# bobu36000/gym-chess

Measured on AMD Instinct MI355X. Metric: env steps/sec at 65 536 boards per GPU (random-policy self-play to terminal, auto-reset), higher is better.
Workload: dtype u64

## Files before the change

### __graft_entry__.py

```python
import os
import subprocess
import sys

ROOT = os.path.dirname(os.path.abspath(__file__))
PKG_DIR = os.path.join(ROOT, "gym-chess_amd")
LIB = os.path.join(PKG_DIR, "gym_chess_amd", "libgymchess.so")
CORE_HOST = os.path.join(ROOT, "tests", "core_host")


def _run(cmd):
    print("+", " ".join(cmd), flush=True)
    subprocess.run(cmd, check=True)


def _lib_module():
    sys.path.insert(0, PKG_DIR)
    from gym_chess_amd import _lib

    return _lib


def build_hip(force=False):
    L = _lib_module()
    want = L.source_hash()
    if not force and os.path.exists(LIB) and L.built_hash(LIB) == want:
        return
    tmp = LIB + ".tmp"
    _run(["hipcc"] + L.BUILD_FLAGS + [f'-DGC_SRC_HASH="{want}"', "-o", tmp,
                                      os.path.join(PKG_DIR, "csrc", "gymchess.hip")])
    os.replace(tmp, LIB)


def build_oracle():
    _run(["make", "-s", "-C", os.path.join(ROOT, "oracle")])


def build_core_host():
    sys.path.insert(0, CORE_HOST)
    import clonehost
    import corehost
    import rankfillhost

    corehost.ensure_built()
    rankfillhost.ensure_built()
    clonehost.ensure_built()


def build():
    build_hip()
    build_oracle()
    build_core_host()
    sys.path.insert(0, PKG_DIR)
    import gym_chess_amd
    from gym_chess_amd import _lib

    _lib.load()


def smoke():
    sys.path.insert(0, PKG_DIR)
    sys.path.insert(0, os.path.join(ROOT, "oracle"))
    import numpy as np

    import oracle as O
    from gym_chess_amd.engine import Engine
    from gym_chess_amd.env import BatchedChessEnv

    eng = Engine(0)
    b = np.tile(O.DEFAULT_BOARD, (64, 1))
    m = np.tile(O.make_meta(), (64, 1))
    nodes = eng.perft(b, m, 3)
    assert (nodes == 8982).all(), nodes[:4]
    moves, cnt = eng.possible_moves(b[:1], m[:1], True)
    assert [int(x) for x in moves[0, : cnt[0]]] == O.get_possible_moves(O.DEFAULT_BOARD, O.make_meta(), True)
    env = BatchedChessEnv(32, device=0, seed=7)
    _, tr = env.rollout(60, trace=True)
    for i in range(32):
        ref = O.rollout_trace(7, i, 60)
        assert (tr["action"][:, i] == ref["action"]).all(), f"board {i} actions differ"
        assert (tr["reward"][:, i] == ref["reward"]).all(), f"board {i} rewards differ"
        assert (tr["done"][:, i] == ref["done"]).all(), f"board {i} done differs"
    print("smoke ok: perft(3)=8982 x64, startpos list, 32x60-ply rollout == oracle", flush=True)


if __name__ == "__main__":
    build()
    if len(sys.argv) > 1 and sys.argv[1] == "smoke":
        smoke()
```

### gym-chess_amd/csrc/gc_core.h

```cpp
#pragma once
#include <type_traits>
#include <stdint.h>

#if defined(__HIPCC__)
#include <hip/hip_runtime.h>
#define GC_HD __host__ __device__ __forceinline__
#define GC_HDM __host__ __device__ __forceinline__
#else
#define GC_HD static inline
#define GC_HDM inline
#endif

namespace gc {

typedef uint64_t u64;
typedef uint32_t u32;

enum { EMPTY = 0, KING = 1, QUEEN = 2, ROOK = 3, BISHOP = 4, KNIGHT = 5, PAWN = 6 };
enum { A_KSW = 4096, A_QSW = 4097, A_KSB = 4098, A_QSB = 4099, A_RESIGN = 4100, A_NONE = 0xFFFF };

enum : u32 {
    M_WHITE = 1u, M_WKC = 2u, M_WQC = 4u, M_BKC = 8u, M_BQC = 16u, M_RIGHTS = 30u,
    M_WCHK = 32u, M_BCHK = 64u, M_DONE = 128u,
    M_MC_SHIFT = 8, M_MC_MASK = 0xFFu << 8,
// ... 1231 lines not shown
            return sq * 64 + (g.white ? sq - 9 : sq + 7);
        }
        return sq * 64 + kth_target(rtg, sq, type_at(s, sq), g.white, k);
    }
    if (g.castles & 1) { if (k == 0) return g.white ? A_QSW : A_QSB; k--; }
    if (g.castles & 2) { if (k == 0) return g.white ? A_KSW : A_KSB; }
    return A_NONE;
}

GC_HD bool action_legal(const Pos& s, const Gen& g, int action) {
    if (action < 0 || action > A_RESIGN) return false;
    if (action >= 4096) {
        if (g.white) return (action == A_QSW && (g.castles & 1)) || (action == A_KSW && (g.castles & 2));
        return (action == A_QSB && (g.castles & 1)) || (action == A_KSB && (g.castles & 2));
    }
    int f = action >> 6, t = action & 63;
    if (!((g.own >> f) & 1)) return false;
    return (legal_targets(s, g, f, type_at(s, f)) >> t) & 1;
}

GC_HD bool quick_legal(const Pos& s, int action) {
    if (action < 0 || action > A_RESIGN) return false;
    Gen g;
    gen_base(s, g);
    if (action >= 4096) {
        gen_enemy(s, g);
        return action_legal(s, g, action);
    }
    const int f = action >> 6, t = action & 63;
    if (!((g.own >> f) & 1)) return false;
    const int ty = type_at(s, f);
    if (ty == KING) return ((king_set(bit(f)) & ~g.own) >> t & 1) && !sq_attacked(s, t, !g.white);
    gen_pins(s, g);
    return (legal_targets(s, g, f, ty) >> t) & 1;
}

GC_HD bool quick_pseudo(const Pos& s, int action) {
    if (action < 0 || action > A_RESIGN) return false;
    Gen g;
    gen_base(s, g);
    if (action >= 4096) {
        gen_enemy(s, g);
        return action_legal(s, g, action);
    }
    const int f = action >> 6, t = action & 63;
    const u64 fb = bit(f), tb = bit(t);
    const int ty = type_at(s, f);
    const int df = (t & 7) - (f & 7), dr = (t >> 3) - (f >> 3);
    const bool orth = (df == 0) != (dr == 0);
    const bool dia = df != 0 && (df == dr || df == -dr);
    const bool clear = (between(f, t) & g.occ) == 0;
    const u64 empty = ~g.occ;
    const u64 push = g.white ? (((fb >> 8) | ((fb & ROW6) >> 16)) & empty) : (((fb << 8) | ((fb & ROW1) << 16)) & empty);
    const u64 pawn = push | (pawn_att_set(fb, g.white) & g.opp);
    const u64 leap = (ty == KNIGHT ? knight_set(fb) : king_set(fb)) & ~g.own;
    const bool ok = ty == PAWN ? (pawn & tb) != 0
                  : (ty == KNIGHT || ty == KING) ? (leap & tb) != 0
                  : ty == QUEEN ? (orth || dia) && clear
                  : ty == ROOK ? orth && clear
                  : ty == BISHOP ? dia && clear : false;
    return ((g.own >> f) & 1) && ok && (ty == PAWN || !(g.own & tb));
}
GC_HD bool quick_safe(const Pos& s, int action) {
    if (action < 0 || action >= 4096) return true;
    const int f = action >> 6, t = action & 63;
    Gen g;
    gen_base(s, g);
    if (type_at(s, f) == KING) return !sq_attacked(s, t, !g.white);
    gen_pins(s, g);
    if (g.ks < 0) return true;
    u64 tg = g.checkmask;
    if (g.pinned & bit(f)) tg &= g.pinrays & line_through(g.ks, f) & king_side(g.ks, f);
    return (tg >> t) & 1;
}

GC_HD int apply_move(Pos& s, bool white_player, int action, int* reward, bool* irrev) {
    *reward = 0;
    *irrev = false;
    if (action < 4096) {
        int f = action >> 6, t = action & 63;
        int pid = id_at(s, f);
        if (pid == 0) return -1;
        int cid = id_at(s, t);
        int pt = pid < 0 ? -pid : pid, ct = cid < 0 ? -cid : cid;
        clear_sq(s, f);
        clear_sq(s, t);
        int nid = pid;
        *reward = (int)((0x1335A00u >> (4 * ct)) & 0xFu);
        if (pt == PAWN && ((white_player && (t >> 3) == 7) || (!white_player && (t >> 3) == 0))) {
            nid = white_player ? QUEEN : -QUEEN;
            *reward += 10;
        }
        put(s, t, nid);
        *irrev = (pt == PAWN) || (cid != 0);
        if (pid == KING) {
            s.meta &= white_player ? ~(u32)(M_WKC | M_WQC) : ~(u32)(M_BKC | M_BQC);
        } else if (pid == ROOK) {
            if ((f & 7) == 0) s.meta &= white_player ? ~(u32)M_WQC : ~(u32)M_BQC;
            else if ((f & 7) == 7) s.meta &= white_player ? ~(u32)M_WKC : ~(u32)M_BKC;
        }
    } else {
        switch (action) {
            case A_KSW:
                clear_sq(s, 60); clear_sq(s, 61); clear_sq(s, 62); clear_sq(s, 63);
                put(s, 61, ROOK); put(s, 62, KING);
                s.meta &= ~(u32)(M_WKC | M_WQC);
                break;
            case A_QSW:
                clear_sq(s, 56); clear_sq(s, 57); clear_sq(s, 58); clear_sq(s, 59); clear_sq(s, 60);
                put(s, 58, KING); put(s, 59, ROOK);
                s.meta &= ~(u32)(M_WKC | M_WQC);
                break;
            case A_KSB:
                clear_sq(s, 4); clear_sq(s, 5); clear_sq(s, 6); clear_sq(s, 7);
                put(s, 5, -ROOK); put(s, 6, -KING);
                s.meta &= ~(u32)(M_BKC | M_BQC);
                break;
            case A_QSB:
                clear_sq(s, 0); clear_sq(s, 1); clear_sq(s, 2); clear_sq(s, 3); clear_sq(s, 4);
                put(s, 2, -KING); put(s, 3, -ROOK);
                s.meta &= ~(u32)(M_BKC | M_BQC);
                break;
            default: return -2;
        }
    }
    s.meta = white_player ? (s.meta & ~(u32)M_WHITE) : (s.meta | M_WHITE);
    return 0;
}

GC_HD void apply_legal_with(Pos& s, bool white, int action, int* reward, bool* irrev, u64 occ0, u64 kw, u64 rw) {
    const bool cs = action >= 4096;
    const bool cw = action == A_KSW || action == A_QSW, cks = action == A_KSW || action == A_KSB;
    const int base = cw ? 56 : 0;
    const u64 cclr = cks ? (0xFull << (base + 4)) : (0x1Full << base);
    const u64 ck = cs ? bit(base + (cks ? 6 : 2)) : 0ull, cr = cs ? bit(base + (cks ? 5 : 3)) : 0ull;
    int f = (action >> 6) & 63, t = action & 63;
    u64 fm = cs ? 0ull : bit(f), tm = cs ? 0ull : bit(t), clr = cs ? ~cclr : ~(fm | tm);
    int v = 10 * (int)((s.q >> t) & 1) + 5 * (int)((s.r >> t) & 1) + 3 * (int)(((s.b | s.n) >> t) & 1) +
            (int)((s.p >> t) & 1);
    *reward = cs ? 0 : v;
    *irrev = !cs && (((s.p & fm) != 0) || ((occ0 & tm) != 0));
    bool wk = (kw & fm) != 0, wr = (rw & fm) != 0;
#define GC_MV(X) s.X = (s.X & clr) | ((s.X & fm) ? tm : 0ull)
    GC_MV(k); GC_MV(q); GC_MV(r); GC_MV(b); GC_MV(n); GC_MV(p); GC_MV(w);
#undef GC_MV
    s.k |= ck;
    s.r |= cr;
    s.w |= cw ? (ck | cr) : 0ull;
    u32 clear = (wk ? (u32)(M_WKC | M_WQC) : 0u) | ((wr && (f & 7) == 0) ? (u32)M_WQC : 0u) |
                ((wr && (f & 7) == 7) ? (u32)M_WKC : 0u);
    clear = cs ? (cw ? (u32)(M_WKC | M_WQC) : (u32)(M_BKC | M_BQC)) : clear;
    s.meta = (s.meta & ~clear) ^ M_WHITE;
}
GC_HD void apply_legal(Pos& s, bool white, int action, int* reward, bool* irrev) {
    apply_legal_with(s, white, action, reward, irrev, occ_of(s), s.k & s.w, s.r & s.w);
}

GC_HD u64 mix64(u64 x) {
    x ^= x >> 31; x *= 0x7FB5D329728EA185ull;
    x ^= x >> 27; x *= 0x81DADEF4BC2DD44Dull;
    x ^= x >> 33;
    return x;
}
GC_HD u64 rotl64(u64 x, int r) { return (x << r) | (x >> (64 - r)); }
GC_HD u32 rotl32(u32 x, int r) { return (x << r) | (x >> (32 - r)); }
GC_HD u32 board_key(const Pos& s) {
    const u64 x = s.k ^ rotl64(s.q, 11) ^ rotl64(s.r, 22) ^ rotl64(s.b, 37) ^ rotl64(s.n, 46) ^ rotl64(s.p, 55) ^
                  rotl64(s.w, 5);
    u32 y = ((u32)x * 0x9E3779B1u) ^ rotl32((u32)(x >> 32) * 0x85EBCA77u, 16);
    y ^= y >> 15;
    y *= 0x2C1B3C6Du;
    return y ^ (y >> 12);
}

GC_HD Pos from_mailbox(const int8_t* b, u32 meta) {
    Pos s = {0, 0, 0, 0, 0, 0, 0, meta};
    for (int i = 0; i < 64; i++) put(s, i, b[i]);
    return s;
}
GC_HD void to_mailbox(const Pos& s, int8_t* b) {
    for (int i = 0; i < 64; i++) b[i] = (int8_t)id_at(s, i);
}

GC_HD u32 philox_x0(u64 seed, u32 board, u32 draw) {
    u32 k0 = (u32)seed, k1 = (u32)(seed >> 32);
    u32 x0 = board, x1 = draw, x2 = 0x5EEDu, x3 = 0u;
#pragma unroll
    for (int i = 0; i < 10; i++) {
        u64 p0 = (u64)0xD2511F53u * x0;
        u64 p1 = (u64)0xCD9E8D57u * x2;
        u32 y0 = (u32)(p1 >> 32) ^ x1 ^ k0;
        u32 y1 = (u32)p1;
        u32 y2 = (u32)(p0 >> 32) ^ x3 ^ k1;
        u32 y3 = (u32)p0;
        x0 = y0; x1 = y1; x2 = y2; x3 = y3;
        k0 += 0x9E3779B9u;
        k1 += 0xBB67AE85u;
    }
    return x0;
}
GC_HD u32 scale_rank(u32 x0, u32 n) { return (u32)(((u64)x0 * n) >> 32); }
GC_HD u32 policy_index(u64 seed, u32 board, u32 draw, u32 n) { return scale_rank(philox_x0(seed, board, draw), n); }

}
```

### gym-chess_amd/csrc/gymchess.hip

```cpp
#include <hip/hip_runtime.h>
#include <hipcub/hipcub.hpp>

#include <cmath>
#include <cstdio>
#include <cstdlib>
#include <cstring>
#include <atomic>
#include <chrono>
#include <mutex>
#include <string>
#include <type_traits>
#include <vector>

#ifdef GC_STAMPS
__shared__ unsigned long long gc_stamp_lds[4][8];
__device__ __forceinline__ void gc_stamp(int k) {
    __builtin_amdgcn_sched_barrier(0);
    unsigned long long t;
#ifdef GC_STAMPS_REAL
    asm volatile("s_memrealtime %0\n\ts_waitcnt lgkmcnt(0)" : "=s"(t)::"memory");
    if (k == 0) {
        unsigned hw, xcc;
        asm volatile("s_getreg_b32 %0, hwreg(HW_REG_HW_ID)\n\ts_getreg_b32 %1, hwreg(HW_REG_XCC_ID)"
                     : "=s"(hw), "=s"(xcc));
// ... 1634 lines not shown
        } else {
            h.commit();
            io.store(i, s);
            h.flush(g0);
            io.nsteps[i] = nst;
            io.reward[i] = o.reward;
            io.done[i] = (uint8_t)o.done;
            io.reason[i] = (uint8_t)o.reason;
        }
    }
    GC_STAMP(7);
#ifdef GC_STAMPS
    if (g_stamp_out != nullptr && l == 0)
        for (int q = 0; q < 8; q++) g_stamp_out[((size_t)blk * 2 + role) * 8 + q] = gc_stamp_lds[threadIdx.x >> 6][q];
#endif
}


__device__ __forceinline__ u64 trace_word(int played, const StepOut& o) {
    return (u64)(uint16_t)(int16_t)played | ((u64)(uint16_t)(int16_t)o.reward << 16) | ((u64)(o.done & 0xFF) << 32) |
           ((u64)(o.reason & 0xFF) << 40);
}
#define ROLLOUT_MAX_PLIES 16383

#ifdef GC_PSTAMPS
__device__ __forceinline__ unsigned long long pst_entry_where() {
    const unsigned long long t = __builtin_amdgcn_s_memrealtime();
    unsigned hw, xcc;
    asm volatile("s_getreg_b32 %0, hwreg(HW_REG_HW_ID)\n\ts_getreg_b32 %1, hwreg(HW_REG_XCC_ID)" : "=s"(hw), "=s"(xcc));
    const unsigned long long where = ((hw >> 8) & 0xF) | (((hw >> 12) & 1) << 4) | (((hw >> 13) & 3) << 5) |
                                     (((hw >> 4) & 3) << 7) | ((unsigned long long)(xcc & 0xF) << 9);
    return (t & ((1ull << 44) - 1)) | (where << 44);
}
#endif

template <bool FIDE, int OPP = 0>
__global__ void __launch_bounds__(2 * PAIR_BOARDS * PAIRS_WG) PAIR_ATTR
    k_env_rollout2(uint8_t* __restrict__ slab, int nn, uint64_t seed, u64* __restrict__ htab,
                   const uint16_t* __restrict__ racts, const EnvDev::InitCache* __restrict__ icd, u32 rinfo,
                   uint64_t* __restrict__ stats, u64* __restrict__ trace) {
    constexpr bool API = false;
    constexpr int blk0 = 0;
    const int plies = (int)(rinfo >> 18);
    rinfo &= 0x1FFFFu;
#ifdef GC_PSTAMPS
    const unsigned long long g_pst_entry = pst_entry_where();
#endif
    PAIR_PROLOGUE
    uint64_t steps = 0, rsum = 0;
    u32 e_mate = 0, e_rep = 0, e_cap = 0, e_nomove = 0, e_err = 0;
    StepOut o = {0, 0, R_NONE, 0};
#ifdef GC_PSTAMPS
    unsigned long long rt0 = 0, rt1 = 0;
    if (l == 0) {
        for (int k = 0; k < 8; k++) gc_pst[threadIdx.x >> 6][k] = 0;
        gc_pst[threadIdx.x >> 6][8] = __builtin_amdgcn_s_memtime();
    }
    rt0 = __builtin_amdgcn_s_memrealtime();
#endif
    const int wg_half = ((nn + PAIR_BOARDS * PAIRS_WG - 1) / (PAIR_BOARDS * PAIRS_WG)) >> 1;
    auto plies_loop = [&](auto R, auto ST) {
        for (int p = 0; p < plies; p++) {
            int played = a;
            if (GC_PAIR_FAIR) {
                if ((((int)blockIdx.x >= wg_half) ? 1 : 0) ^ (p & 1)) __builtin_amdgcn_s_setprio(1);
                else __builtin_amdgcn_s_setprio(0);
            }
            o = pair_step<OPP, true, FIDE>(Ls, L, C, R, l, i, live, rp, s, a, d, h, nst);
#ifdef GC_PSTAMPS
            if (p == 0) rt1 = __builtin_amdgcn_s_memrealtime();
#endif
            if (R) {
                if (trace && live) trace[(size_t)p * nn + i] = trace_word(played == A_NONE ? -1 : played, o);
                if (!ST) {
                } else if (played == A_NONE) {
                    e_nomove++;
                } else {
                    steps++;
                    rsum += (uint64_t)(int64_t)o.reward;
                    if (o.done) {
                        e_mate += o.reason == R_MATE || o.reason == R_MATED;
                        e_rep += o.reason == R_REPETITION;
                        e_cap += o.reason == R_MOVE_CAP;
                        e_err += o.reason == R_BOTH_CHECKED || o.reason == R_WINDOW_FULL;
                        e_nomove += o.reason == R_OPP_NO_MOVE;
                    }
                }
                h.commit();
            }
        }
#ifdef GC_PSTAMPS
        if (g_pst_out != nullptr && l == 0) {
            const size_t w = (size_t)blockIdx.x * (blockDim.x >> 6) + (threadIdx.x >> 6);
            for (int k = 0; k < 8; k++) g_pst_out[w * 12 + k] = gc_pst[threadIdx.x >> 6][k];
            g_pst_out[w * 12 + 8] = g_pst_entry;
            g_pst_out[w * 12 + 9] = rt0;
            g_pst_out[w * 12 + 10] = rt1;
            g_pst_out[w * 12 + 11] = __builtin_amdgcn_s_memrealtime();
        }
#endif
        const PairIO io = store_io(slab, nn);
        if (live) {
            if (R == 0) {
                io.act[i] = (uint16_t)a;
                io.draw[i] = d;
            } else {
                io.store(i, s);
                h.flush(g0);
                io.nsteps[i] = nst;
                io.reward[i] = o.reward;
                io.done[i] = (uint8_t)o.done;
                io.reason[i] = (uint8_t)o.reason;
                if (ST) {
                    uint64_t* so = stats + 8 * (size_t)i;
                    so[0] += steps; so[1] += rsum;
                    so[2 + R_MATE] += e_mate; so[2 + R_REPETITION] += e_rep; so[2 + R_MOVE_CAP] += e_cap;
                    so[2 + R_NO_MOVES] += e_nomove; so[2 + R_BOTH_CHECKED] += e_err;
                }
            }
        }
    };
    if (role == 0) plies_loop(RoleC<0>{}, std::false_type{});
    else if (stats) plies_loop(RoleC<1>{}, std::true_type{});
    else plies_loop(RoleC<1>{}, std::false_type{});
}

#define QUAD_BOARDS 64
#ifndef QUADS_WG
#define QUADS_WG 2
#endif
#ifndef GC_QXOR
#define GC_QXOR 2
#endif
#define ROLL_QUADS_WG 1

struct QuadLds {
    u64 sets[SW_SETS][QUAD_BOARDS];
    u64 ns[NBB][QUAD_BOARDS];
    u32 nmeta[QUAD_BOARDS];
    int32_t mr[QUAD_BOARDS];
    u32 irrev[QUAD_BOARDS];
    u64 pin3[3][QUAD_BOARDS];
    u32 f0[QUAD_BOARDS];
    u64 enemy[3][QUAD_BOARDS];
    u32 f1[QUAD_BOARDS];
    u64 cwx[2][4][QUAD_BOARDS];
    u64 cw0[2][QUAD_BOARDS];
    u32 part[4][QUAD_BOARDS];
    u32 rep[QUAD_BOARDS];
    u32 x0[QUAD_BOARDS];
    u32 ra[QUAD_BOARDS];
    u32 act[QUAD_BOARDS];
    u32 pick[QUAD_BOARDS];
    u32 castles[QUAD_BOARDS];
    u64 occ[HTAB / 64][QUAD_BOARDS];
    u32 nkey[QUAD_BOARDS];
    u32 rkey0;
    Pos rp;
};
template <class LT>
struct QuadSetsT {
    LT& L;
    int l;
    u64 cw[4];
    int part;
    __device__ void put(int j, u64 t) {
        L.sets[j][l] = t;
        const int c = popc(t);
        cw[j >> 3] |= (u64)c << (8 * (j & 7));
        part += c;
    }
    template <int LO, int HI>
    __device__ void put_all(const u64* t) {
#pragma unroll
        for (int j = LO; j < HI; j++) put(j, t[j - LO]);
    }
};
using QuadSets = QuadSetsT<QuadLds>;

struct QuadPend {
    bool have;
    uint16_t ra;
    __device__ int resolve(const QuadLds& L, int l) const {
        const int pk = (int)L.pick[l];
        return have ? pk : (int)ra;
    }
};
struct QuadQ0Pre {
    u32 meta0;
    u64 occ, kw, rw;
};
__device__ __forceinline__ QuadQ0Pre quad_q0pre(const Pos& s) {
    QuadQ0Pre q{(s.meta & ~(u32)M_RIGHTS) | eff_rights(s), occ_of(s), s.k & s.w, s.r & s.w};
    pin(q.meta0); pin(q.occ); pin(q.kw); pin(q.rw);
    return q;
}

struct OccQ {
    bool valid;
    bool clr;
    bool probe;
    bool fast;
};
#ifndef GC_WG_FAIR
#define GC_WG_FAIR 1
#endif
#ifndef GC_OCC_RUN
#define GC_OCC_RUN 1
#endif
#define QSETPRIO(x, up)                                       \
    do {                                                      \
        if (GC_WG_FAIR && (up)) __builtin_amdgcn_s_setprio((x) + 1); \
        else __builtin_amdgcn_s_setprio(x);                   \
    } while (0)
template <int R, bool OCC>
__device__ __forceinline__ StepOut quad_ply(QuadLds& L, const PairCtx& C, int l, int i, bool live, Pos& s, int& a,
                                            u32& d, DevHist& h, u32& nst, RepProbe& pr, QuadPend& pend, OccQ& oq,
                                            QuadQ0Pre& q0, bool up = false) {
    constexpr bool CARRY = R < 2;
#ifdef GC_PSTAMPS
    bool pst_loaded = false;
#endif
    if (R == 0) QSETPRIO(2, up);
    if (R == 2) QSETPRIO(0, up);
    if (GC_WG_FAIR && R == 1) QSETPRIO(2, up);
    if (GC_WG_FAIR && R == 3) QSETPRIO(0, up);
    if (R == 0) a = pend.resolve(L, l);
    u32 x0 = 0;
    uint16_t ra = (uint16_t)A_NONE;
    if (R == 1) {
        x0 = philox_x0(C.seed, (u32)i, d);
        if (C.rtable) ra = C.racts[scale_rank(x0, C.rtotal)];
        L.x0[l] = x0;
    }
    if (R == 0) L.act[l] = (u32)a;
    PST(7);
    if (R == 1) {
        pair_barrier();
        a = (int)L.act[l];
    }
    const bool none = a == A_NONE;
    const bool done0 = (s.meta & M_DONE) != 0;
    const bool cap = mc_of(s.meta) > MOVES_MAX;
    const bool mv = live && !none && !done0 && !cap;
    const bool white = (s.meta & M_WHITE) != 0;
    int mr = 0;
    bool irrev = false;
    Pos ns;
    if (R == 0) {
        ns = s;
        ns.meta = q0.meta0;
        if (mv) apply_legal_with(ns, white, a, &mr, &irrev, q0.occ, q0.kw, q0.rw);
        L.ns[0][l] = ns.k; L.ns[1][l] = ns.q; L.ns[2][l] = ns.r; L.ns[3][l] = ns.b;
        L.ns[4][l] = ns.n; L.ns[5][l] = ns.p; L.ns[6][l] = ns.w;
        L.nmeta[l] = ns.meta;
        L.mr[l] = mr;
        L.irrev[l] = irrev ? 1u : 0u;
    }
    PST(0);
    if (R != 1) pair_barrier();
    PST(1);
    Gen g;
    bool my_chk = false;
    OrthCarry oc{};
    DiagCarry dc{};
    if (R != 0) {
        ns.k = L.ns[0][l]; ns.q = L.ns[1][l]; ns.r = L.ns[2][l]; ns.b = L.ns[3][l];
        ns.n = L.ns[4][l]; ns.p = L.ns[5][l]; ns.w = L.ns[6][l];
        ns.meta = L.nmeta[l];
    }
    if (R == 1) {
        mr = L.mr[l];
        irrev = L.irrev[l] != 0;
    }
    gen_base(ns, g);
    if (R == 0) {
        gen_pins(ns, g);
        L.pin3[0][l] = g.checkmask;
        L.pin3[1][l] = g.pinned;
        L.pin3[2][l] = g.pinrays;
        L.f0[l] = g.in_check ? 1u : 0u;
    } else if (R == 1) {
        my_chk = mv && mover_checked(s, ns, white, a);
        L.f1[l] = my_chk ? 1u : 0u;
        if constexpr (OCC) {
        if (oq.clr) {
#pragma unroll
            for (int w = 0; w < HTAB / 64; w++) L.occ[w][l] = 0ull;
            oq.clr = false;
        }
        const u32 nk = board_key(ns);
        L.nkey[l] = nk;
        oq.probe = !oq.valid || ((L.occ[(nk & (HTAB - 1)) >> 6][l] >> (nk & 63)) & 1) != 0;
        }
    } else if (R == 2) {
        oc = orth_carry(g.occ);
        L.enemy[1][l] = g.ks >= 0 ? side_attacks_leapers(ns, !g.white) | side_attacks_orth(ns, !g.white, oc) : 0ull;
    } else {
        dc = diag_carry(g.occ);
        L.enemy[2][l] = g.ks >= 0 ? side_attacks_diag(ns, !g.white, dc) : 0ull;
    }
    PST(2);
    pair_barrier();
    PST(3);
#define QUAD_ENEMY(l) (L.enemy[1][l] | L.enemy[2][l])
    if (R == 0) {
        g.enemy_att = QUAD_ENEMY(l);
        gen_castles(ns, g);
        my_chk = L.f1[l] != 0;
    } else if (R == 1) {
        g.in_check = L.f0[l] != 0;
    } else {
        g.checkmask = L.pin3[0][l];
        g.pinned = L.pin3[1][l];
        g.pinrays = L.pin3[2][l];
        if (R == 2) g.enemy_att = QUAD_ENEMY(l);
    }
    const bool opp_chk = g.in_check;
    const bool both = opp_chk && my_chk;
    const bool gen = mv && !both;
    QuadSets Q{L, l, {0, 0, 0, 0}, 0};
    int c = 0;
    u32 hl = hl_of(s.meta);
    if (R == 0) {
        if (gen) {
            u64 T[SW_SETS];
            sw_pawns(ns, g, T);
            Q.put_all<SW_P1, SW_N>(T + SW_P1);
            sw_knights(ns, g, T);
            Q.put_all<SW_N, SW_ORTH>(T + SW_N);
            Q.part += popc(g.castles);
        }
        L.cw0[0][l] = Q.cw[0];
        L.cw0[1][l] = Q.cw[1];
        L.castles[l] = g.castles;
    } else if (R == 1) {
        if (mv && !both) {
            pin(pr.e0.hdr); pin(pr.e0.k); pin(pr.e0.q); pin(pr.e0.r);
            pin(pr.e0.b); pin(pr.e0.n); pin(pr.e0.p); pin(pr.e0.w);
            if (OCC && oq.fast) pr.e0.hdr = (u64)(h.gen() ^ 1u);
            if constexpr (OCC && GC_OCC_RUN) {
                c = rep_commit(h, s, pr, hl, irrev, [&](u32 pos) {
                    const bool free = oq.valid && ((L.occ[pos >> 6][l] >> (pos & 63)) & 1) == 0;
                    PST_LOADED(!free);
                    return free;
                });
            } else {
                c = rep_commit(h, s, pr, hl, irrev, [&](u32) {
                    PST_LOADED(true);
                    return false;
                });
            }
            if (!OCC) {
            } else if (irrev) {
                oq.valid = true;
                oq.clr = true;
                oq.probe = false;
            } else if (h.wkind == 2) {
                L.occ[h.wpos >> 6][l] |= 1ull << (h.wpos & 63);
                oq.probe = oq.probe || (u32)h.wpos == (L.nkey[l] & (HTAB - 1));
            }
        }
        L.rep[l] = (u32)c | (hl << 8);
        L.ra[l] = ra;
    } else if (R == 2) {
        u64 T[SW_SETS];
        sw_orth(ns, g, oc, T);
        Q.put_all<SW_ORTH, SW_DIAG>(T + SW_ORTH);
        sw_kings(ns, g, T);
        Q.put_all<SW_K, SW_SETS>(T + SW_K);
        L.part[2][l] = (u32)Q.part;
#pragma unroll
        for (int k = 0; k < 4; k++) L.cwx[0][k][l] = Q.cw[k];
    } else {
        u64 T[SW_SETS];
        sw_diag(ns, g, dc, T);
        Q.put_all<SW_DIAG, SW_K>(T + SW_DIAG);
        L.part[3][l] = (u32)Q.part;
#pragma unroll
        for (int k = 0; k < 4; k++) L.cwx[1][k][l] = Q.cw[k];
    }
    if (R == 0) L.part[0][l] = (u32)Q.part;
#ifdef GC_PSTAMPS
    if (R == 1) gc_pst_mark_run(4, pst_loaded);
    else
#endif
    PST(4);
    pair_barrier();
    PST(5);
    StepOut o = {0, 0, R_NONE, 0};
    if (R == 0) QSETPRIO(0, up);
    if (R == 2) QSETPRIO(2, up);
    if (R == 2) {
        const int total = (int)L.part[0][l] + Q.part + (int)L.part[3][l];
        u64 cw[4];
#pragma unroll
        for (int k = 0; k < 4; k++) cw[k] = Q.cw[k] | L.cwx[1][k][l];
        cw[0] |= L.cw0[0][l];
        cw[1] |= L.cw0[1][l];
        g.castles = L.castles[l];
        L.pick[l] = total > 0 ? (u32)sw_pick_lds(L, l, g, cw, total, (int)scale_rank(L.x0[l], (u32)total)) : (u32)A_NONE;
    }
    if constexpr (CARRY) {
        const int total = gen ? (R == 0 ? Q.part : (int)L.part[0][l]) + (int)L.part[2][l] + (int)L.part[3][l] : 0;
        if (R == 0) {
            const u32 rpk = L.rep[l];
            c = (int)(rpk & 0xFFu);
            hl = rpk >> 8;
            ra = (uint16_t)L.ra[l];
        } else {
            h.commit();
        }
        bool have = false;
        if (none) {
            o.reason = R_NO_MOVES;
        } else {
            nst += 1;
            if (done0) { o.done = 1; o.reason = R_DONE_ALREADY; }
            else if (cap) { o.done = 1; o.reason = R_MOVE_CAP; }
            else if (both) { o.done = 1; o.reason = R_BOTH_CHECKED; }
            else {
                const u32 chk = white ? ((my_chk ? M_WCHK : 0u) | (opp_chk ? M_BCHK : 0u))
                                      : ((opp_chk ? M_WCHK : 0u) | (my_chk ? M_BCHK : 0u));
                s = ns;
                s.meta = with_hl((ns.meta & ~(u32)(M_WCHK | M_BCHK | M_DONE)) | chk | ((c >= 3 || c == 0) ? M_DONE : 0u), hl);
                o.reward = -10 + mr;
                o.moved = 1;
                if (c >= 3) { o.done = 1; o.reason = R_REPETITION; }
                if (c == 0) { o.done = 1; o.reason = R_WINDOW_FULL; }
                if (total == 0 && opp_chk) {
                    s.meta |= M_DONE;
                    o.done = 1;
                    o.reward += 100;
                    o.reason = R_MATE;
                }
                if (!o.done && !white) s.meta += (1u << M_MC_SHIFT);
                have = true;
            }
            if (o.done) have = false;
        }
        if (!have) {
            s = L.rp;
            h.bump_gen();
        }
        if (R == 1 && OCC) {
            pr.key = have ? L.nkey[l] : L.rkey0;
            if (!have) {
                oq.valid = true;
                oq.clr = true;
            }
            oq.fast = !(live && have && oq.probe);
            const ulonglong2* src = oq.fast ? reinterpret_cast<const ulonglong2*>(C.icd)
                                            : reinterpret_cast<const ulonglong2*>(h.htab + h.entry((int)(pr.key & (HTAB - 1))) * 8);
            const ulonglong2 e0 = src[0], e1 = src[1], e2 = src[2], e3 = src[3];
            pr.e0 = RepEntry{e0.x, e0.y, e1.x, e1.y, e2.x, e2.y, e3.x, e3.y};
        } else if (R == 1 && live) {
            rep_prefetch(h, s, pr);
        }
        const int tot = have ? total : (int)C.rtotal;
        d += tot > 0 ? 1u : 0u;
        if (R == 0) {
            pend = QuadPend{have, ra};
            q0 = quad_q0pre(s);
        }
    }
    PST(6);
    pair_barrier();
    return o;
}

__shared__ QuadLds g_quad_lds[ROLL_QUADS_WG];
__shared__ QuadLds g_quad_lds2[QUADS_WG];
template <int QW>
__device__ __forceinline__ QuadLds& roll_lds(int qw) {
    if constexpr (QW == ROLL_QUADS_WG) return g_quad_lds[qw];
    else return g_quad_lds2[qw];
}

#define ROLL_TURNS 0xCA69C6A9C69AC69Cull
template <int QW>
__device__ __forceinline__ int roll_place(int block, int wgs) {
    const int part = wgs / (4 / QW);
    return (part ? block / part : block) & (4 / QW - 1);
}
template <int QW>
__device__ __forceinline__ bool roll_turn(int place, int turn) {
    if (QW == 2) return ((place ^ turn) & 1) != 0;
    return ((ROLL_TURNS >> (4 * (turn & 15) + place)) & 1) != 0;
}

template <int RR, bool ST, bool OCC, int QW>
__device__ __forceinline__ void quad_run(uint8_t* __restrict__ slab, int nn, uint64_t seed, u64* __restrict__ htab,
                                      const uint16_t* __restrict__ racts, const EnvDev::InitCache* __restrict__ icd,
                                      u32 rinfo, int plies, uint64_t* __restrict__ stats, u64* __restrict__ trace,
                                      int qw, int l, int i, int place) {
    QuadLds& L = roll_lds<QW>(qw);
    const bool live = i < nn;
    const int ii = live ? i : nn - 1;
    const PairIO in_io(slab, nn);
    const PairCtx C = {seed, htab, in_io.hgen, racts, icd, (rinfo >> 16) != 0, rinfo & 0xFFFFu};
    Pos s{};
    u32 ua = 0, g0 = 0, nst = 0, d = 0;
    if (RR < 2) {
        s = in_io.load(ii);
        ua = in_io.act[ii];
        g0 = in_io.hgen[ii];
        nst = in_io.nsteps[ii];
        d = in_io.draw[ii];
        pin(s); pin(ua); pin(g0); pin(nst); pin(d);
    }
    if (RR == 3 && l == 0) {
        const Pos rp = icd->pos;
        L.rp = rp;
        if (OCC) L.rkey0 = board_key(rp);
    }
    int a = (int)ua;
    DevHist h = DevHist{htab, in_io.hgen, g0, ii, HTAB_BITS};
    RepProbe pr;
    if (RR == 1 && live) rep_prefetch(h, s, pr);
    OccQ oq{RR == 1 && hl_of(s.meta) == 0, RR == 1, true, false};
    QuadPend pend{false, (uint16_t)ua};
    QuadQ0Pre q0{};
    if (RR == 0) q0 = quad_q0pre(s);
#ifdef GC_PSTAMPS
    const unsigned long long g_pst_entry = pst_entry_where();
    unsigned long long rt1 = 0;
    if (l == 0) {
        for (int k = 0; k < 8; k++) gc_pst[threadIdx.x >> 6][k] = 0;
        gc_pst_run[threadIdx.x >> 6][0] = gc_pst_run[threadIdx.x >> 6][1] = 0;
        gc_pst[threadIdx.x >> 6][8] = __builtin_amdgcn_s_memtime();
    }
    const unsigned long long rt0 = __builtin_amdgcn_s_memrealtime();
#endif
    u32 sa = 0, sb = 0, sc = 0;
    int32_t rsum = 0;
    StepOut o = {0, 0, R_NONE, 0};
#ifndef GC_TURN_SHIFT
#define GC_TURN_SHIFT 2
#endif
    constexpr int TURN = 1 << GC_TURN_SHIFT;
    for (int p0 = 0; p0 < plies; p0 += TURN) {
      const bool up = GC_WG_FAIR && roll_turn<QW>(place, p0 >> GC_TURN_SHIFT);
      const int pe = p0 + TURN < plies ? p0 + TURN : plies;
      for (int p = p0; p < pe; p++) {
        o = quad_ply<RR, OCC>(L, C, l, i, live, s, a, d, h, nst, pr, pend, oq, q0, up);
        const int played = a;
#ifdef GC_PSTAMPS
        if (p == 0) rt1 = __builtin_amdgcn_s_memrealtime();
#endif
        if (RR == 1) {
            if (trace && live) trace[(size_t)p * nn + i] = trace_word(played == A_NONE ? -1 : played, o);
            if (!ST) {
            } else if (played == A_NONE) {
                sc += 1u << 16;
            } else {
                sa += 1u;
                rsum += o.reward;
                if (o.done) {
                    sb += (o.reason == R_MATE || o.reason == R_MATED ? 1u : 0u) | (o.reason == R_REPETITION ? 1u << 16 : 0u);
                    sc += (o.reason == R_MOVE_CAP ? 1u : 0u) | (o.reason == R_OPP_NO_MOVE ? 1u << 16 : 0u);
                    sa += o.reason == R_BOTH_CHECKED || o.reason == R_WINDOW_FULL ? 1u << 16 : 0u;
                }
            }
            h.commit();
        }
      }
    }
#ifdef GC_PSTAMPS
    if (g_pst_out != nullptr && l == 0) {
        const size_t w = (size_t)blockIdx.x * (blockDim.x >> 6) + (threadIdx.x >> 6);
        for (int k = 0; k < 8; k++) g_pst_out[w * 12 + k] = gc_pst[threadIdx.x >> 6][k];
        g_pst_out[w * 12 + 8] = g_pst_entry;
        g_pst_out[w * 12 + 9] = rt0;
        g_pst_out[w * 12 + 10] = rt1;
        g_pst_out[w * 12 + 11] = __builtin_amdgcn_s_memrealtime();
        if (g_pst_run_out != nullptr) {
            g_pst_run_out[w * 2] = gc_pst_run[threadIdx.x >> 6][0];
            g_pst_run_out[w * 2 + 1] = gc_pst_run[threadIdx.x >> 6][1];
        }
    }
#endif
    if (!live || RR >= 2) return;
    const PairIO io = store_io(slab, nn);
    if (RR == 0) {
        a = pend.resolve(L, l);
        io.act[i] = (uint16_t)a;
        io.draw[i] = d;
    } else {
        io.store(i, s);
        if (h.gen() != g0) io.hgen[i] = h.gen();
        io.nsteps[i] = nst;
        io.reward[i] = o.reward;
        io.done[i] = (uint8_t)o.done;
        io.reason[i] = (uint8_t)o.reason;
        if (ST) {
            uint64_t* so = stats + 8 * (size_t)i;
            so[0] += sa & 0xFFFFu; so[1] += (uint64_t)(int64_t)rsum;
            so[2 + R_MATE] += sb & 0xFFFFu; so[2 + R_REPETITION] += sb >> 16; so[2 + R_MOVE_CAP] += sc & 0xFFFFu;
            so[2 + R_NO_MOVES] += sc >> 16; so[2 + R_BOTH_CHECKED] += sa >> 16;
        }
    }
}

template <bool OCC, int QW>
__global__ void __launch_bounds__(4 * QUAD_BOARDS * QW) __attribute__((amdgpu_waves_per_eu(4)))
    k_env_rollout4(uint8_t* __restrict__ slab, int nn, uint64_t seed, u64* __restrict__ htab,
                   const uint16_t* __restrict__ racts, const EnvDev::InitCache* __restrict__ icd, u32 rinfo,
                   uint64_t* __restrict__ stats, u64* __restrict__ trace) {
    const int plies = (int)(rinfo >> 18);
    rinfo &= 0x1FFFFu;
    const int wv = __builtin_amdgcn_readfirstlane((int)(threadIdx.x >> 6));
    const int qw = wv >> 2;
    const int wgs = (nn + QUAD_BOARDS * QW - 1) / (QUAD_BOARDS * QW);
    const int place = roll_place<QW>((int)blockIdx.x, wgs);
    const int role = (wv & 3) ^ ((qw & 1) ? GC_QXOR : 0);
    const int l = threadIdx.x & (QUAD_BOARDS - 1);
    const int i = (blockIdx.x * QW + qw) * QUAD_BOARDS + l;
#ifndef GC_QPRIO
#define GC_QPRIO 0x0A
#endif
    switch ((GC_QPRIO >> (2 * role)) & 3) {
        case 1: __builtin_amdgcn_s_setprio(1); break;
        case 2: __builtin_amdgcn_s_setprio(2); break;
        case 3: __builtin_amdgcn_s_setprio(3); break;
        default: break;
    }
    switch (role) {
        case 0: quad_run<0, false, OCC, QW>(slab, nn, seed, htab, racts, icd, rinfo, plies, stats, trace, qw, l, i, place); break;
        case 1:
            if (stats) quad_run<1, true, OCC, QW>(slab, nn, seed, htab, racts, icd, rinfo, plies, stats, trace, qw, l, i, place);
            else quad_run<1, false, OCC, QW>(slab, nn, seed, htab, racts, icd, rinfo, plies, stats, trace, qw, l, i, place);
            break;
        case 2: quad_run<2, false, OCC, QW>(slab, nn, seed, htab, racts, icd, rinfo, plies, stats, trace, qw, l, i, place); break;
        default: quad_run<3, false, OCC, QW>(slab, nn, seed, htab, racts, icd, rinfo, plies, stats, trace, qw, l, i, place); break;
    }
    const EnvDev::InitCache::DoneWord dw = icd->done;
    if (dw.ctr) {
        __syncthreads();
        if (threadIdx.x == 0) {
            const u32 prev = __hip_atomic_fetch_add(dw.ctr, 1u, __ATOMIC_RELAXED, __HIP_MEMORY_SCOPE_AGENT);
            if (prev == (u32)wgs - 1) {
                __hip_atomic_store(dw.ctr, 0u, __ATOMIC_RELAXED, __HIP_MEMORY_SCOPE_AGENT);
                const u32 v = __hip_atomic_fetch_add(dw.seq, 1u, __ATOMIC_RELAXED, __HIP_MEMORY_SCOPE_AGENT) + 1u;
                __hip_atomic_store(dw.host, v, __ATOMIC_RELAXED, __HIP_MEMORY_SCOPE_SYSTEM);
            }
        }
    }
}

template <bool OPP>
__global__ void __launch_bounds__(BLOCK) k_env_rollout(EnvDev e, int plies, u64* trace, uint64_t* stats) {
    LDS_SCRATCH_DECL;
    int i = blockIdx.x * blockDim.x + threadIdx.x;
    if (i >= e.n) return;
    Pos s = e.st.load(i);
    u32 g0 = e.hgen[i], d = e.draw[i], ua = e.act[i];
    pin(s); pin(g0); pin(d); pin(ua);
    DevHist h = e.hist(i, g0);
    PolicyCtx pc = {e.seed, (u32)i, d};
    int a = (int)ua;
    uint64_t steps = 0, rsum = 0;
    u32 e_mate = 0, e_rep = 0, e_cap = 0, e_nomove = 0, e_err = 0;
    StepOut o = {0, 0, R_NONE, 0};
    for (int p = 0; p < plies; p++) {
        o = {0, 0, R_NONE, 0};
        Gen g;
        MoveSet ms;
        bool have = false;
        int played = a;
        if (a == A_NONE) {
            reset_board(e, s, h);
            o.reason = R_NO_MOVES;
            e_nomove++;
            played = -1;
        } else {
            o = OPP ? env_step_vs<false>(s, h, a, nullptr, g, ms, scr, pc) : env_step<false>(s, h, a, nullptr, g, ms, scr);
            have = o.moved;
            steps++;
            rsum += (uint64_t)(int64_t)o.reward;
            if (o.done) {
                e_mate += o.reason == R_MATE || o.reason == R_MATED;
                e_rep += o.reason == R_REPETITION;
                e_cap += o.reason == R_MOVE_CAP;
                e_err += o.reason == R_BOTH_CHECKED || o.reason == R_WINDOW_FULL;
                e_nomove += o.reason == R_OPP_NO_MOVE;
                reset_board(e, s, h);
                have = false;
            }
        }
        if (OPP && !have) after_reset<OPP>(e, s, h, g, ms, scr, pc);
        if (trace) trace[(size_t)p * e.n + i] = trace_word(played, o);
        a = selfplay_pick(s, pc);
        h.commit();
    }
    e.reward[i] = o.reward;
    e.done[i] = (uint8_t)o.done;
    e.reason[i] = (uint8_t)o.reason;
    e.st.store(i, s);
// ... 1766 lines not shown
```

Baseline: 18.78 billion.

## Split move application across two waves and precompute random draw ahead

Under a new S0 mode, used when the quad count equals the per-workgroup maximum, applying a move is split. One wave updates the king, rook, white and meta bitboards, and another updates the queen, bishop, knight and pawn bitboards along with reward and irreversibility. The results are exchanged through LDS. Wave 3 now computes the philox draw and random-table action one ply ahead, writes them to LDS, and recomputes them only when the draw counter it reads from LDS differs from its own. This is meant to shorten the critical path of each ply by balancing work across waves and removing the act handoff barrier. The cost is more LDS traffic, extra state to keep in sync, and a risk of divergence when the speculated draw is wrong.

```diff
diff --git a/__graft_entry__.py b/__graft_entry__.py
--- a/__graft_entry__.py
+++ b/__graft_entry__.py
@@ -37,6 +37,7 @@
 
 def build_core_host():
     sys.path.insert(0, CORE_HOST)
+    import applysplithost
     import clonehost
     import corehost
     import rankfillhost
@@ -44,6 +45,7 @@
     corehost.ensure_built()
     rankfillhost.ensure_built()
     clonehost.ensure_built()
+    applysplithost.ensure_built()
 
 
 def build():
diff --git a/gym-chess_amd/csrc/gc_core.h b/gym-chess_amd/csrc/gc_core.h
--- a/gym-chess_amd/csrc/gc_core.h
+++ b/gym-chess_amd/csrc/gc_core.h
@@ -1407,6 +1407,44 @@
     clear = cs ? (cw ? (u32)(M_WKC | M_WQC) : (u32)(M_BKC | M_BQC)) : clear;
     s.meta = (s.meta & ~clear) ^ M_WHITE;
 }
+struct ApplyMasks {
+    bool cs, cw;
+    u64 fm, tm, clr;
+    u64 ck, cr;
+};
+GC_HD ApplyMasks apply_masks(int action) {
+    const bool cs = action >= 4096;
+    const bool cw = action == A_KSW || action == A_QSW, cks = action == A_KSW || action == A_KSB;
+    const int base = cw ? 56 : 0;
+    const u64 cclr = cks ? (0xFull << (base + 4)) : (0x1Full << base);
+    const u64 ck = cs ? bit(base + (cks ? 6 : 2)) : 0ull, cr = cs ? bit(base + (cks ? 5 : 3)) : 0ull;
+    const u64 fm = cs ? 0ull : bit((action >> 6) & 63), tm = cs ? 0ull : bit(action & 63);
+    return ApplyMasks{cs, cw, fm, tm, cs ? ~cclr : ~(fm | tm), ck, cr};
+}
+#define GC_MV(X) s.X = (s.X & m.clr) | ((s.X & m.fm) ? m.tm : 0ull)
+GC_HD void apply_legal_krw(Pos& s, int action, u64 kw, u64 rw) {
+    const ApplyMasks m = apply_masks(action);
+    const int f = (action >> 6) & 63;
+    const bool wk = (kw & m.fm) != 0, wr = (rw & m.fm) != 0;
+    GC_MV(k); GC_MV(r); GC_MV(w);
+    s.k |= m.ck;
+    s.r |= m.cr;
+    s.w |= m.cw ? (m.ck | m.cr) : 0ull;
+    u32 clear = (wk ? (u32)(M_WKC | M_WQC) : 0u) | ((wr && (f & 7) == 0) ? (u32)M_WQC : 0u) |
+                ((wr && (f & 7) == 7) ? (u32)M_WKC : 0u);
+    clear = m.cs ? (m.cw ? (u32)(M_WKC | M_WQC) : (u32)(M_BKC | M_BQC)) : clear;
+    s.meta = (s.meta & ~clear) ^ M_WHITE;
+}
+GC_HD void apply_legal_qbnp(Pos& s, int action, int* reward, bool* irrev, u64 occ0) {
+    const ApplyMasks m = apply_masks(action);
+    const int t = action & 63;
+    const int v = 10 * (int)((s.q >> t) & 1) + 5 * (int)((s.r >> t) & 1) + 3 * (int)(((s.b | s.n) >> t) & 1) +
+                  (int)((s.p >> t) & 1);
+    *reward = m.cs ? 0 : v;
+    *irrev = !m.cs && (((s.p & m.fm) != 0) || ((occ0 & m.tm) != 0));
+    GC_MV(q); GC_MV(b); GC_MV(n); GC_MV(p);
+}
+#undef GC_MV
 GC_HD void apply_legal(Pos& s, bool white, int action, int* reward, bool* irrev) {
     apply_legal_with(s, white, action, reward, irrev, occ_of(s), s.k & s.w, s.r & s.w);
 }
diff --git a/gym-chess_amd/csrc/gymchess.hip b/gym-chess_amd/csrc/gymchess.hip
--- a/gym-chess_amd/csrc/gymchess.hip
+++ b/gym-chess_amd/csrc/gymchess.hip
@@ -1810,6 +1810,7 @@
     u32 ra[QUAD_BOARDS];
     u32 act[QUAD_BOARDS];
     u32 pick[QUAD_BOARDS];
+    u32 d[QUAD_BOARDS];
     u32 castles[QUAD_BOARDS];
     u64 occ[HTAB / 64][QUAD_BOARDS];
     u32 nkey[QUAD_BOARDS];
@@ -1848,10 +1849,24 @@
     u32 meta0;
     u64 occ, kw, rw;
 };
+template <bool S0>
 __device__ __forceinline__ QuadQ0Pre quad_q0pre(const Pos& s) {
-    QuadQ0Pre q{(s.meta & ~(u32)M_RIGHTS) | eff_rights(s), occ_of(s), s.k & s.w, s.r & s.w};
-    pin(q.meta0); pin(q.occ); pin(q.kw); pin(q.rw);
+    QuadQ0Pre q{(s.meta & ~(u32)M_RIGHTS) | eff_rights(s), S0 ? 0ull : occ_of(s), s.k & s.w, s.r & s.w};
+    pin(q.meta0); pin(q.kw); pin(q.rw);
+    if (!S0) pin(q.occ);
     return q;
+}
+__device__ __forceinline__ QuadQ0Pre quad_q1pre(const Pos& s) {
+    QuadQ0Pre q{0u, occ_of(s), 0ull, 0ull};
+    pin(q.occ);
+    return q;
+}
+struct QuadAhead {
+    u32 x0, ra;
+};
+__device__ __forceinline__ void quad_ahead(const PairCtx& C, int i, u32 d, QuadAhead& ah) {
+    ah.x0 = philox_x0(C.seed, (u32)i, d);
+    ah.ra = C.rtable ? (u32)C.racts[scale_rank(ah.x0, C.rtotal)] : (u32)(uint16_t)A_NONE;
 }
 
 struct OccQ {
@@ -1871,10 +1886,10 @@
         if (GC_WG_FAIR && (up)) __builtin_amdgcn_s_setprio((x) + 1); \
         else __builtin_amdgcn_s_setprio(x);                   \
     } while (0)
-template <int R, bool OCC>
+template <int R, bool OCC, bool S0>
 __device__ __forceinline__ StepOut quad_ply(QuadLds& L, const PairCtx& C, int l, int i, bool live, Pos& s, int& a,
                                             u32& d, DevHist& h, u32& nst, RepProbe& pr, QuadPend& pend, OccQ& oq,
-                                            QuadQ0Pre& q0, bool up = false) {
+                                            QuadQ0Pre& q0, QuadAhead& ah, bool up = false) {
     constexpr bool CARRY = R < 2;
 #ifdef GC_PSTAMPS
     bool pst_loaded = false;
@@ -1883,17 +1898,26 @@
     if (R == 2) QSETPRIO(0, up);
     if (GC_WG_FAIR && R == 1) QSETPRIO(2, up);
     if (GC_WG_FAIR && R == 3) QSETPRIO(0, up);
-    if (R == 0) a = pend.resolve(L, l);
+    if (R == 0 || (S0 && R == 1)) a = pend.resolve(L, l);
     u32 x0 = 0;
     uint16_t ra = (uint16_t)A_NONE;
-    if (R == 1) {
+    if (R == 1 && !S0) {
         x0 = philox_x0(C.seed, (u32)i, d);
         if (C.rtable) ra = C.racts[scale_rank(x0, C.rtotal)];
         L.x0[l] = x0;
     }
-    if (R == 0) L.act[l] = (u32)a;
+    if (R == 3 && S0) {
+        const u32 dt = L.d[l];
+        if (__any(dt != d)) {
+            d = dt;
+            quad_ahead(C, i, d, ah);
+        }
+        L.x0[l] = ah.x0;
+        L.ra[l] = ah.ra;
+    }
+    if (R == 0 && !S0) L.act[l] = (u32)a;
     PST(7);
-    if (R == 1) {
+    if (R == 1 && !S0) {
         pair_barrier();
         a = (int)L.act[l];
     }
@@ -1905,7 +1929,17 @@
     int mr = 0;
     bool irrev = false;
     Pos ns;
-    if (R == 0) {
+    if (R == 0 && S0) {
+        ns = s;
+        ns.meta = q0.meta0;
+        if (mv) apply_legal_krw(ns, a, q0.kw, q0.rw);
+        L.ns[0][l] = ns.k; L.ns[2][l] = ns.r; L.ns[6][l] = ns.w;
+        L.nmeta[l] = ns.meta;
+    } else if (R == 1 && S0) {
+        ns = s;
+        if (mv) apply_legal_qbnp(ns, a, &mr, &irrev, q0.occ);
+        L.ns[1][l] = ns.q; L.ns[3][l] = ns.b; L.ns[4][l] = ns.n; L.ns[5][l] = ns.p;
+    } else if (R == 0) {
         ns = s;
         ns.meta = q0.meta0;
         if (mv) apply_legal_with(ns, white, a, &mr, &irrev, q0.occ, q0.kw, q0.rw);
@@ -1916,18 +1950,23 @@
         L.irrev[l] = irrev ? 1u : 0u;
     }
     PST(0);
-    if (R != 1) pair_barrier();
+    if (R != 1 || S0) pair_barrier();
     PST(1);
     Gen g;
     bool my_chk = false;
     OrthCarry oc{};
     DiagCarry dc{};
-    if (R != 0) {
+    if (R == 0 && S0) {
+        ns.q = L.ns[1][l]; ns.b = L.ns[3][l]; ns.n = L.ns[4][l]; ns.p = L.ns[5][l];
+    } else if (R == 1 && S0) {
+        ns.k = L.ns[0][l]; ns.r = L.ns[2][l]; ns.w = L.ns[6][l];
+        ns.meta = L.nmeta[l];
+    } else if (R != 0) {
         ns.k = L.ns[0][l]; ns.q = L.ns[1][l]; ns.r = L.ns[2][l]; ns.b = L.ns[3][l];
         ns.n = L.ns[4][l]; ns.p = L.ns[5][l]; ns.w = L.ns[6][l];
         ns.meta = L.nmeta[l];
     }
-    if (R == 1) {
+    if (R == 1 && !S0) {
         mr = L.mr[l];
         irrev = L.irrev[l] != 0;
     }
@@ -2020,7 +2059,7 @@
             }
         }
         L.rep[l] = (u32)c | (hl << 8);
-        L.ra[l] = ra;
+        if (!S0) L.ra[l] = ra;
     } else if (R == 2) {
         u64 T[SW_SETS];
         sw_orth(ns, g, oc, T);
@@ -2067,6 +2106,7 @@
             hl = rpk >> 8;
             ra = (uint16_t)L.ra[l];
         } else {
+            if (S0) ra = (uint16_t)L.ra[l];
             h.commit();
         }
         bool have = false;
@@ -2118,9 +2158,18 @@
         const int tot = have ? total : (int)C.rtotal;
         d += tot > 0 ? 1u : 0u;
         if (R == 0) {
+            if (S0) L.d[l] = d;
             pend = QuadPend{have, ra};
-            q0 = quad_q0pre(s);
-        }
+            q0 = quad_q0pre<S0>(s);
+        } else if (S0) {
+            pend = QuadPend{have, ra};
+            q0 = quad_q1pre(s);
+        }
+    }
+    if (R == 3 && S0) {
+        d += 1u;
+        pin(d);
+        quad_ahead(C, i, d, ah);
     }
     PST(6);
     pair_barrier();
@@ -2152,6 +2201,7 @@
                                       const uint16_t* __restrict__ racts, const EnvDev::InitCache* __restrict__ icd,
                                       u32 rinfo, int plies, uint64_t* __restrict__ stats, u64* __restrict__ trace,
                                       int qw, int l, int i, int place) {
+    constexpr bool S0 = QW == ROLL_QUADS_WG;
     QuadLds& L = roll_lds<QW>(qw);
     const bool live = i < nn;
     const int ii = live ? i : nn - 1;
@@ -2159,6 +2209,10 @@
     const PairCtx C = {seed, htab, in_io.hgen, racts, icd, (rinfo >> 16) != 0, rinfo & 0xFFFFu};
     Pos s{};
     u32 ua = 0, g0 = 0, nst = 0, d = 0;
+    if (RR == 3 && S0) {
+        d = in_io.draw[ii];
+        pin(d);
+    }
     if (RR < 2) {
         s = in_io.load(ii);
         ua = in_io.act[ii];
@@ -2179,7 +2233,13 @@
     OccQ oq{RR == 1 && hl_of(s.meta) == 0, RR == 1, true, false};
     QuadPend pend{false, (uint16_t)ua};
     QuadQ0Pre q0{};
-    if (RR == 0) q0 = quad_q0pre(s);
+    if (RR == 0) q0 = quad_q0pre<S0>(s);
+    if (RR == 1 && S0) q0 = quad_q1pre(s);
+    QuadAhead ah{};
+    if (RR == 3 && S0) {
+        quad_ahead(C, i, d, ah);
+        L.d[l] = d;
+    }
 #ifdef GC_PSTAMPS
     const unsigned long long g_pst_entry = pst_entry_where();
     unsigned long long rt1 = 0;
@@ -2201,7 +2261,7 @@
       const bool up = GC_WG_FAIR && roll_turn<QW>(place, p0 >> GC_TURN_SHIFT);
       const int pe = p0 + TURN < plies ? p0 + TURN : plies;
       for (int p = p0; p < pe; p++) {
-        o = quad_ply<RR, OCC>(L, C, l, i, live, s, a, d, h, nst, pr, pend, oq, q0, up);
+        o = quad_ply<RR, OCC, S0>(L, C, l, i, live, s, a, d, h, nst, pr, pend, oq, q0, ah, up);
         const int played = a;
 #ifdef GC_PSTAMPS
         if (p == 0) rt1 = __builtin_amdgcn_s_memrealtime();
```

Measured after the change: 19.58 billion (median of 6 runs). +4.3%, better.
